# evenrose/CMDIAD

Measured on AMD Instinct MI355X. Metric: images/sec end-to-end (extract+distill+kNN score), higher is better.
Workload: dtype bf16; 1 GPU; configs[1]: DINO ViT-B/8 + Point-MAE predict (DoubleRGBPointFeatures: both modalities are extracted, this method has no distillation step at test time; the `mtfi_step` leg times the method that has one), 224x224 RGB + 24576-point clouds (1024 groups x 128), batch 32/GPU, bagel-sized banks (xyz 76518x768, rgb 19129x768); batch_per_gpu=32, rotating_input_batches=4, bank=single, hip_graphs=True, search_operands=bf16 (fp32 accumulate, exact fp32 re-score of the winner), weights=seeded random init (no checkpoints offline)

## Files before the change

### cmdiad_amd/csrc/mlp_fused.hip

```cpp
#include "gemm_core.h"
#include "launch.h"

namespace {

using namespace gemm;

constexpr int kC = 384, kHid = 1536, kBM = 128, kWaves = 8;
constexpr int kChunks = kHid / 64;
constexpr int kKT1 = kC / BK;
constexpr int kPer = kKT1 + kC / 64;
constexpr int kSlots = 6, kAhead = kSlots - 1;
static_assert(kPer % kSlots == 0, "the slot of a piece depends on its place in the chunk only");
constexpr int kPieceBytes = 64 * BK * 2;
constexpr int kXbWave = kKT1 * 16 * BK * 2;
constexpr int kHOff = kWaves * kXbWave;
constexpr int kRingOff = kHOff + kWaves * 2048;
constexpr int kLdsBytes = kRingOff + kSlots * kPieceBytes;
static_assert(kLdsBytes == 160 * 1024, "LDS budget");

struct MlpParams {
    int M;
    const bf16_t* xb;
    const float* row_scale;
    const bf16_t* w1;
    const float* b1;
    const bf16_t* w2;
    const float* b2;
    float* x;
    bf16_t* ln_xb;
    float* ln_part;
    const float* add2;
};

__device__ __forceinline__ void mlp_barrier() { asm volatile("s_barrier" ::: "memory"); }

__device__ __forceinline__ float half_row_sum8(float v)
{
    v += __builtin_bit_cast(float, __builtin_amdgcn_update_dpp(0, __builtin_bit_cast(int, v), 0xB1, 0xF, 0xF, false));
    v += __builtin_bit_cast(float, __builtin_amdgcn_update_dpp(0, __builtin_bit_cast(int, v), 0x4E, 0xF, 0xF, false));
    v += __builtin_bit_cast(float, __builtin_amdgcn_update_dpp(0, __builtin_bit_cast(int, v), 0x141, 0xF, 0xF, false));
    return v;
}

template <bool LN_OUT>
__global__ __launch_bounds__(512, 1) void pmae_mlp_fused_kernel(MlpParams p)
{
    extern __shared__ __attribute__((aligned(16))) char lds[];
    const int lane = threadIdx.x & 63, wave = __builtin_amdgcn_readfirstlane(threadIdx.x >> 6);
    const int g = lane >> 4, r16 = lane & 15;
    const int mw = (int)blockIdx.x * kBM + wave * 16;
    char* xs = lds + wave * kXbWave;
    char* hs = lds + kHOff + wave * 2048;
    char* ring = lds + kRingOff;

    float rsc;
    f32x4 b1v[4];
    auto load_b1 = [&](int c) {
        const float* bp = p.b1 + c * 64 + g * 4;
#pragma unroll
        for (int j = 0; j < 4; ++j) asm volatile("global_load_dwordx4 %0, %1, off" : "=v"(b1v[j]) : "v"(bp + j * 16) : "memory");
    };
    {
        const float* rp = p.row_scale + min(mw + r16, p.M - 1);
        asm volatile("global_load_dword %0, %1, off" : "=v"(rsc) : "v"(rp) : "memory");
    }
    load_b1(0);
    const int sw_chunk = (lane & 7) ^ (lane >> 3);
#pragma unroll
    for (int e = 0; e < 2; ++e) {
        const bf16_t* src = p.xb + (size_t)min(mw + e * 8 + (lane >> 3), p.M - 1) * kC + sw_chunk * 8;
#pragma unroll
        for (int s = 0; s < kKT1; ++s)
            __builtin_amdgcn_global_load_lds((const __attribute__((address_space(1))) void*)(src + s * BK),
                                             (__attribute__((address_space(3))) void*)(xs + s * 2048 + e * 1024), 16, 0, 0);
    }
    const char* w1l = reinterpret_cast<const char*>(p.w1 + (size_t)(wave * 8 + (lane >> 3)) * kC + sw_chunk * 8);
    const char* w2l = reinterpret_cast<const char*>(p.w2 + (size_t)(wave * 8 + (lane >> 3)) * kHid + sw_chunk * 8);
    auto issue = [&](int c, int q) {
        const char* src = q < kKT1 ? w1l + ((size_t)c * 64 * kC + q * BK) * 2 : w2l + ((size_t)(q - kKT1) * 64 * kHid + c * BK) * 2;
        __builtin_amdgcn_global_load_lds((const __attribute__((address_space(1))) void*)src,
                                         (__attribute__((address_space(3))) void*)(ring + (q % kSlots) * kPieceBytes + wave * 1024), 16, 0, 0);
    };
#pragma unroll
    for (int q = 0; q < kAhead; ++q) issue(0, q);
    asm volatile("s_waitcnt vmcnt(4)" ::: "memory");
    mlp_barrier();

    auto ldf = [&](const char* tile, int row, int kk) { return *reinterpret_cast<const bf16x8*>(tile + lds_off(row, kk * 4 + g)); };
    auto step = [&](const char* wt, const bf16x8& a0, const bf16x8& a1, f32x4 (&acc)[4]) {
        bf16x8 wf[2][4];
#pragma unroll
        for (int kk = 0; kk < 2; ++kk)
#pragma unroll
            for (int j = 0; j < 4; ++j) wf[kk][j] = ldf(wt, j * 16 + r16, kk);
        __builtin_amdgcn_s_setprio(1);
#pragma unroll
        for (int kk = 0; kk < 2; ++kk)
#pragma unroll
            for (int j = 0; j < 4; ++j) acc[j] = mfma16(wf[kk][j], kk ? a1 : a0, acc[j]);
        __builtin_amdgcn_s_setprio(0);
    };

    f32x4 acc2[kC / 64][4];
#pragma unroll
    for (int nb = 0; nb < kC / 64; ++nb)
#pragma unroll
        for (int j = 0; j < 4; ++j) acc2[nb][j] = f32x4{0.f, 0.f, 0.f, 0.f};

    for (int c = 0; c < kChunks; ++c) {
        f32x4 acc1[4];
#pragma unroll
        for (int j = 0; j < 4; ++j) acc1[j] = f32x4{0.f, 0.f, 0.f, 0.f};
        bf16x8 h0, h1;
#pragma unroll
        for (int q = 0; q < kPer; ++q) {
            const int qn = q + kAhead < kPer ? q + kAhead : q + kAhead - kPer;
            const int cn = q + kAhead < kPer ? c : c + 1;
            const bool more = cn < kChunks;
            if (q == 7 && more) load_b1(c + 1);
            if (more) issue(cn, qn);
            const char* wt = ring + (q % kSlots) * kPieceBytes;
            if (q < kKT1) step(wt, ldf(xs + q * 2048, r16, 0), ldf(xs + q * 2048, r16, 1), acc1);
            else step(wt, h0, h1, acc2[q - kKT1]);
            if (!more) asm volatile("s_waitcnt vmcnt(0)" ::: "memory");
            else if (q >= 7 && q <= 10) asm volatile("s_waitcnt vmcnt(8)" ::: "memory");
            else asm volatile("s_waitcnt vmcnt(4)" ::: "memory");
            mlp_barrier();
            if (q == kKT1 - 1) {
                __builtin_amdgcn_sched_barrier(0);
#pragma unroll
                for (int j = 0; j < 4; ++j) {
                    f32x4 v = __builtin_elementwise_fma(acc1[j], f32x4{rsc, rsc, rsc, rsc}, b1v[j]);
                    v = gelu_erf4(v);
                    const bf16x4 hv = {f2bf(v[0]), f2bf(v[1]), f2bf(v[2]), f2bf(v[3])};
                    *reinterpret_cast<bf16x4*>(hs + lds_off(r16, 2 * j + (g >> 1)) + (g & 1) * 8) = hv;
                }
                h0 = ldf(hs, r16, 0);
                h1 = ldf(hs, r16, 1);
            }
        }
    }

    RowStore32 rs;
    rs.init(hs, lane);
    const bool full = mw + 16 <= p.M;
    const int m0r = mw + rs.R;
    const int ma = min(m0r, p.M - 1), mb = min(m0r + 8, p.M - 1);
#pragma unroll
    for (int nb = 0; nb < kC / 64; ++nb) {
        const int n0 = nb * 64;
        f32x4 bj[4];
#pragma unroll
        for (int j = 0; j < 4; ++j) bj[j] = *reinterpret_cast<const f32x4*>(p.b2 + n0 + j * 16 + g * 4);
        f32x4 o0[2], o1[2];
#pragma unroll
        for (int ch = 0; ch < 2; ++ch) {
            const int col = n0 + ch * 32 + rs.u * 4;
            const f32x4 r0 = *reinterpret_cast<const f32x4*>(p.x + (size_t)ma * kC + col);
            const f32x4 r1 = *reinterpret_cast<const f32x4*>(p.x + (size_t)mb * kC + col);
            f32x4 a0 = {0.f, 0.f, 0.f, 0.f}, a1 = a0;
            if (LN_OUT && p.add2) {
                a0 = *reinterpret_cast<const f32x4*>(p.add2 + (size_t)ma * kC + col);
                a1 = *reinterpret_cast<const f32x4*>(p.add2 + (size_t)mb * kC + col);
            }
            rs.park(acc2[nb][2 * ch] + bj[2 * ch], acc2[nb][2 * ch + 1] + bj[2 * ch + 1]);
            f32x4 t0, t1;
            rs.fetch(t0, t1);
            o0[ch] = t0 + r0;
            o1[ch] = t1 + r1;
            if (LN_OUT && p.add2) { o0[ch] += a0; o1[ch] += a1; }
            if (full || m0r < p.M) *reinterpret_cast<f32x4*>(p.x + (size_t)m0r * kC + col) = o0[ch];
            if (full || m0r + 8 < p.M) *reinterpret_cast<f32x4*>(p.x + (size_t)(m0r + 8) * kC + col) = o1[ch];
            if constexpr (LN_OUT) {
                const bf16x4 v0 = {f2bf(o0[ch][0]), f2bf(o0[ch][1]), f2bf(o0[ch][2]), f2bf(o0[ch][3])};
                const bf16x4 v1 = {f2bf(o1[ch][0]), f2bf(o1[ch][1]), f2bf(o1[ch][2]), f2bf(o1[ch][3])};
                if (full || m0r < p.M) *reinterpret_cast<bf16x4*>(p.ln_xb + (size_t)m0r * kC + col) = v0;
                if (full || m0r + 8 < p.M) *reinterpret_cast<bf16x4*>(p.ln_xb + (size_t)(m0r + 8) * kC + col) = v1;
            }
        }
        if constexpr (LN_OUT) {
            float s0 = 0.f, s1 = 0.f;
#pragma unroll
            for (int ch = 0; ch < 2; ++ch)
#pragma unroll
                for (int q = 0; q < 4; ++q) { s0 += o0[ch][q]; s1 += o1[ch][q]; }
            s0 = half_row_sum8(s0);
            s1 = half_row_sum8(s1);
            const float c0 = s0 * (1.0f / 64), c1 = s1 * (1.0f / 64);
            float q0 = 0.f, q1 = 0.f;
#pragma unroll
            for (int ch = 0; ch < 2; ++ch)
#pragma unroll
                for (int q = 0; q < 4; ++q) {
                    const float d0 = o0[ch][q] - c0, d1 = o1[ch][q] - c1;
                    q0 = fmaf(d0, d0, q0);
                    q1 = fmaf(d1, d1, q1);
                }
            q0 = half_row_sum8(q0);
            q1 = half_row_sum8(q1);
            if (rs.u == 0) {
                float2* part = reinterpret_cast<float2*>(p.ln_part) + (size_t)nb * p.M;
                if (full || m0r < p.M) part[m0r] = make_float2(s0, q0);
                if (full || m0r + 8 < p.M) part[m0r + 8] = make_float2(s1, q1);
            }
        }
    }
}

}

int cmdiad_pmae_mlp_fused(float* x, const uint16_t* xb, const float* rstd, const uint16_t* w1, const float* b1, const uint16_t* w2,
                          const float* b2, int M, uint16_t* ln_xb, float* ln_part, const float* add2, cmdiad_stream_t stream)
{
    CMDIAD_REQUIRE(x && xb && rstd && w1 && b1 && w2 && b2 && M > 0, CMDIAD_ERR_ARG, "cmdiad_pmae_mlp_fused: null operand");
    CMDIAD_REQUIRE(aligned16(x) && aligned16(xb) && aligned16(w1) && aligned16(w2) && aligned16(b1) && aligned16(b2) && (!add2 || aligned16(add2)), CMDIAD_ERR_ARG,
                   "cmdiad_pmae_mlp_fused: operands must be 16-byte aligned");
    CMDIAD_REQUIRE(!ln_xb == !ln_part && (ln_xb || !add2) && (!ln_xb || (((uintptr_t)ln_xb & 7) == 0 && ((uintptr_t)ln_part & 7) == 0)),
                   CMDIAD_ERR_ARG, "cmdiad_pmae_mlp_fused: ln_xb and ln_part come together (8-byte aligned); add2 only with them");
    MlpParams p{M, (const bf16_t*)xb, rstd, (const bf16_t*)w1, b1, (const bf16_t*)w2, b2, x, (bf16_t*)ln_xb, ln_part, add2};
    const dim3 grid((unsigned)((M + kBM - 1) / kBM)), block(kWaves * 64);
    const int rc = ln_xb ? launch_lds<pmae_mlp_fused_kernel<true>>("cmdiad_pmae_mlp_fused", grid, block, kLdsBytes, (hipStream_t)stream, p)
                         : launch_lds<pmae_mlp_fused_kernel<false>>("cmdiad_pmae_mlp_fused", grid, block, kLdsBytes, (hipStream_t)stream, p);
    if (rc) return rc;
    CMDIAD_CHECK_LAUNCH();
    return CMDIAD_OK;
}
```

Measured before the change: 1581 images/s.

## Retile fused Point-MAE MLP into 32x32 wave tiles with double-buffered fragments

Changes the fused FC1-GELU-FC2 kernel so that each wave owns a 32-row by half-width tile instead of 16 full-width rows. The input and hidden tiles become shared across the block, and FC2 output columns are split between wave pairs. The change also double-buffers LDS fragment reads against MFMAs, issues two weight pieces per phase through explicit SGPR-based DMA, and adds lgkmcnt waits before each barrier. The aim is to cut per-MFMA LDS weight traffic and hide LDS latency. In exchange it needs an extra barrier for the shared hidden tile and takes on more register pressure and a trickier ring-slot schedule.

```diff
diff --git a/cmdiad_amd/csrc/mlp_fused.hip b/cmdiad_amd/csrc/mlp_fused.hip
--- a/cmdiad_amd/csrc/mlp_fused.hip
+++ b/cmdiad_amd/csrc/mlp_fused.hip
@@ -9,14 +9,16 @@
 constexpr int kChunks = kHid / 64;
 constexpr int kKT1 = kC / BK;
 constexpr int kPer = kKT1 + kC / 64;
-constexpr int kSlots = 6, kAhead = kSlots - 1;
+constexpr int kSlots = 6;
 static_assert(kPer % kSlots == 0, "the slot of a piece depends on its place in the chunk only");
 constexpr int kPieceBytes = 64 * BK * 2;
-constexpr int kXbWave = kKT1 * 16 * BK * 2;
-constexpr int kHOff = kWaves * kXbWave;
-constexpr int kRingOff = kHOff + kWaves * 2048;
+constexpr int kXbBlock = kBM * BK * 2;
+constexpr int kHOff = kKT1 * kXbBlock;
+constexpr int kHBytes = kBM * 64 * 2;
+constexpr int kRingOff = kHOff + kHBytes;
 constexpr int kLdsBytes = kRingOff + kSlots * kPieceBytes;
 static_assert(kLdsBytes == 160 * 1024, "LDS budget");
+static_assert(kHBytes >= kWaves * 2048, "the hidden tile doubles as the waves' RowStore32 scratch");
 
 struct MlpParams {
     int M;
@@ -32,7 +34,7 @@
     const float* add2;
 };
 
-__device__ __forceinline__ void mlp_barrier() { asm volatile("s_barrier" ::: "memory"); }
+__device__ __forceinline__ void mlp_barrier() { asm volatile("s_waitcnt lgkmcnt(0)\n\ts_barrier" ::: "memory"); }
 
 __device__ __forceinline__ float half_row_sum8(float v)
 {
@@ -48,160 +50,214 @@
     extern __shared__ __attribute__((aligned(16))) char lds[];
     const int lane = threadIdx.x & 63, wave = __builtin_amdgcn_readfirstlane(threadIdx.x >> 6);
     const int g = lane >> 4, r16 = lane & 15;
-    const int mw = (int)blockIdx.x * kBM + wave * 16;
-    char* xs = lds + wave * kXbWave;
-    char* hs = lds + kHOff + wave * 2048;
+    const int tr = wave >> 1, nc = wave & 1;
+    const int m0 = (int)blockIdx.x * kBM;
+    const int mt = m0 + tr * 32;
+    char* xs = lds;
+    char* hs = lds + kHOff;
     char* ring = lds + kRingOff;
 
-    float rsc;
-    f32x4 b1v[4];
+    float rsc[2];
+    f32x4 b1v[2];
     auto load_b1 = [&](int c) {
-        const float* bp = p.b1 + c * 64 + g * 4;
-#pragma unroll
-        for (int j = 0; j < 4; ++j) asm volatile("global_load_dwordx4 %0, %1, off" : "=v"(b1v[j]) : "v"(bp + j * 16) : "memory");
-    };
+        const float* bp = p.b1 + c * 64 + nc * 32 + g * 4;
+#pragma unroll
+        for (int j = 0; j < 2; ++j) asm volatile("global_load_dwordx4 %0, %1, off" : "=v"(b1v[j]) : "v"(bp + j * 16) : "memory");
+    };
+#pragma unroll
+    for (int i = 0; i < 2; ++i) {
+        const float* rp = p.row_scale + min(mt + i * 16 + r16, p.M - 1);
+        asm volatile("global_load_dword %0, %1, off" : "=v"(rsc[i]) : "v"(rp) : "memory");
+    }
+    load_b1(0);
+    auto dma = [&](const char* ubase, unsigned voff, unsigned lds_addr) {
+        unsigned long long sb;
+        asm volatile("s_mov_b64 %0, %2\n\ts_mov_b32 m0, %3\n\ts_nop 0\n\tglobal_load_lds_dwordx4 %1, %0"
+                     : "=&s"(sb) : "v"(voff), "s"(ubase), "s"(lds_addr) : "memory");
+    };
+    const unsigned lds0 = (unsigned)(size_t)(__attribute__((address_space(3))) char*)lds;
+    const unsigned pch = (unsigned)(((lane & 7) ^ (lane >> 3)) * 16);
     {
-        const float* rp = p.row_scale + min(mw + r16, p.M - 1);
-        asm volatile("global_load_dword %0, %1, off" : "=v"(rsc) : "v"(rp) : "memory");
-    }
-    load_b1(0);
-    const int sw_chunk = (lane & 7) ^ (lane >> 3);
-#pragma unroll
-    for (int e = 0; e < 2; ++e) {
-        const bf16_t* src = p.xb + (size_t)min(mw + e * 8 + (lane >> 3), p.M - 1) * kC + sw_chunk * 8;
-#pragma unroll
-        for (int s = 0; s < kKT1; ++s)
-            __builtin_amdgcn_global_load_lds((const __attribute__((address_space(1))) void*)(src + s * BK),
-                                             (__attribute__((address_space(3))) void*)(xs + s * 2048 + e * 1024), 16, 0, 0);
-    }
-    const char* w1l = reinterpret_cast<const char*>(p.w1 + (size_t)(wave * 8 + (lane >> 3)) * kC + sw_chunk * 8);
-    const char* w2l = reinterpret_cast<const char*>(p.w2 + (size_t)(wave * 8 + (lane >> 3)) * kHid + sw_chunk * 8);
+        const char* xb0 = reinterpret_cast<const char*>(p.xb) + (size_t)m0 * kC * 2;
+        const int last = p.M - 1 - m0;
+#pragma unroll
+        for (int e = 0; e < 2; ++e) {
+            const unsigned voff = (unsigned)min(wave * 16 + e * 8 + (lane >> 3), last) * (unsigned)(kC * 2) + pch;
+#pragma unroll
+            for (int s = 0; s < kKT1; ++s) dma(xb0 + s * BK * 2, voff, lds0 + s * kXbBlock + (wave * 16 + e * 8) * 128);
+        }
+    }
+    const unsigned off1 = (unsigned)(wave * 8 + (lane >> 3)) * (unsigned)(kC * 2) + pch;
+    const unsigned off2 = (unsigned)(wave * 8 + (lane >> 3)) * (unsigned)(kHid * 2) + pch;
     auto issue = [&](int c, int q) {
-        const char* src = q < kKT1 ? w1l + ((size_t)c * 64 * kC + q * BK) * 2 : w2l + ((size_t)(q - kKT1) * 64 * kHid + c * BK) * 2;
-        __builtin_amdgcn_global_load_lds((const __attribute__((address_space(1))) void*)src,
-                                         (__attribute__((address_space(3))) void*)(ring + (q % kSlots) * kPieceBytes + wave * 1024), 16, 0, 0);
-    };
-#pragma unroll
-    for (int q = 0; q < kAhead; ++q) issue(0, q);
+        const unsigned dst = lds0 + kRingOff + (q % kSlots) * kPieceBytes + wave * 1024;
+        if (q < kKT1) dma(reinterpret_cast<const char*>(p.w1) + ((size_t)c * 64 * kC + q * BK) * 2, off1, dst);
+        else dma(reinterpret_cast<const char*>(p.w2) + ((size_t)(q - kKT1) * 64 * kHid + c * BK) * 2, off2, dst);
+    };
+#pragma unroll
+    for (int q = 0; q < kSlots; ++q) issue(0, q);
     asm volatile("s_waitcnt vmcnt(4)" ::: "memory");
     mlp_barrier();
 
     auto ldf = [&](const char* tile, int row, int kk) { return *reinterpret_cast<const bf16x8*>(tile + lds_off(row, kk * 4 + g)); };
-    auto step = [&](const char* wt, const bf16x8& a0, const bf16x8& a1, f32x4 (&acc)[4]) {
-        bf16x8 wf[2][4];
+    bf16x8 fx[2][2][2];
+    bf16x8 fw[2][4];
+    bf16x8 hf[2][2];
+    f32x4 acc1[2][2];
+    f32x4 acc2[3][2][4];
+    auto read_fc1 = [&](int h, int s) {
+        const char* xt = xs + s * kXbBlock;
+        const char* wt = ring + s * kPieceBytes;
+#pragma unroll
+        for (int kk = 0; kk < 2; ++kk) {
+#pragma unroll
+            for (int i = 0; i < 2; ++i) fx[h][kk][i] = ldf(xt, tr * 32 + i * 16 + r16, kk);
+#pragma unroll
+            for (int jj = 0; jj < 2; ++jj) fw[h][2 * kk + jj] = ldf(wt, nc * 32 + jj * 16 + r16, kk);
+        }
+    };
+    auto mfma_fc1 = [&](int h) {
+        __builtin_amdgcn_s_setprio(1);
 #pragma unroll
         for (int kk = 0; kk < 2; ++kk)
 #pragma unroll
-            for (int j = 0; j < 4; ++j) wf[kk][j] = ldf(wt, j * 16 + r16, kk);
+            for (int i = 0; i < 2; ++i)
+#pragma unroll
+                for (int jj = 0; jj < 2; ++jj) acc1[i][jj] = mfma16(fw[h][2 * kk + jj], fx[h][kk][i], acc1[i][jj]);
+        __builtin_amdgcn_s_setprio(0);
+    };
+    auto read_fc2 = [&](int kk, int pp) {
+        const char* wt = ring + (2 * pp + nc) * kPieceBytes;
+#pragma unroll
+        for (int j = 0; j < 4; ++j) fw[kk][j] = ldf(wt, j * 16 + r16, kk);
+    };
+    auto mfma_fc2 = [&](int kk, int pp) {
         __builtin_amdgcn_s_setprio(1);
 #pragma unroll
-        for (int kk = 0; kk < 2; ++kk)
-#pragma unroll
-            for (int j = 0; j < 4; ++j) acc[j] = mfma16(wf[kk][j], kk ? a1 : a0, acc[j]);
+        for (int i = 0; i < 2; ++i)
+#pragma unroll
+            for (int j = 0; j < 4; ++j) acc2[pp][i][j] = mfma16(fw[kk][j], hf[kk][i], acc2[pp][i][j]);
         __builtin_amdgcn_s_setprio(0);
     };
 
-    f32x4 acc2[kC / 64][4];
-#pragma unroll
-    for (int nb = 0; nb < kC / 64; ++nb)
-#pragma unroll
-        for (int j = 0; j < 4; ++j) acc2[nb][j] = f32x4{0.f, 0.f, 0.f, 0.f};
-
+#pragma unroll
+    for (int pp = 0; pp < 3; ++pp)
+#pragma unroll
+        for (int i = 0; i < 2; ++i)
+#pragma unroll
+            for (int j = 0; j < 4; ++j) acc2[pp][i][j] = f32x4{0.f, 0.f, 0.f, 0.f};
+
+    read_fc1(0, 0);
     for (int c = 0; c < kChunks; ++c) {
-        f32x4 acc1[4];
-#pragma unroll
-        for (int j = 0; j < 4; ++j) acc1[j] = f32x4{0.f, 0.f, 0.f, 0.f};
-        bf16x8 h0, h1;
-#pragma unroll
-        for (int q = 0; q < kPer; ++q) {
-            const int qn = q + kAhead < kPer ? q + kAhead : q + kAhead - kPer;
-            const int cn = q + kAhead < kPer ? c : c + 1;
-            const bool more = cn < kChunks;
-            if (q == 7 && more) load_b1(c + 1);
-            if (more) issue(cn, qn);
-            const char* wt = ring + (q % kSlots) * kPieceBytes;
-            if (q < kKT1) step(wt, ldf(xs + q * 2048, r16, 0), ldf(xs + q * 2048, r16, 1), acc1);
-            else step(wt, h0, h1, acc2[q - kKT1]);
-            if (!more) asm volatile("s_waitcnt vmcnt(0)" ::: "memory");
-            else if (q >= 7 && q <= 10) asm volatile("s_waitcnt vmcnt(8)" ::: "memory");
-            else asm volatile("s_waitcnt vmcnt(4)" ::: "memory");
+        const bool more = c + 1 < kChunks;
+#pragma unroll
+        for (int i = 0; i < 2; ++i)
+#pragma unroll
+            for (int jj = 0; jj < 2; ++jj) acc1[i][jj] = f32x4{0.f, 0.f, 0.f, 0.f};
+#pragma unroll
+        for (int P = 0; P < 6; ++P) {
+            if (P < 3) { read_fc1(1, 2 * P + 1); __builtin_amdgcn_sched_barrier(0); mfma_fc1(0); }
+            else { read_fc2(1, P - 3); __builtin_amdgcn_sched_barrier(0); mfma_fc2(0, P - 3); }
+            if (P >= 4 && !more) asm volatile("s_waitcnt vmcnt(0)" ::: "memory");
+            else if (P == 4) asm volatile("s_waitcnt vmcnt(4)" ::: "memory");
+            else asm volatile("s_waitcnt vmcnt(2)" ::: "memory");
             mlp_barrier();
-            if (q == kKT1 - 1) {
+            if (P < 3) { issue(c, 2 * P + 6); issue(c, 2 * P + 7); }
+            else if (more) {
+                if (P == 3) load_b1(c + 1);
+                issue(c + 1, 2 * P - 6);
+                issue(c + 1, 2 * P - 5);
+            }
+            if (P < 2) { read_fc1(0, 2 * P + 2); __builtin_amdgcn_sched_barrier(0); mfma_fc1(1); }
+            else if (P == 2) {
+                mfma_fc1(1);
                 __builtin_amdgcn_sched_barrier(0);
 #pragma unroll
-                for (int j = 0; j < 4; ++j) {
-                    f32x4 v = __builtin_elementwise_fma(acc1[j], f32x4{rsc, rsc, rsc, rsc}, b1v[j]);
-                    v = gelu_erf4(v);
-                    const bf16x4 hv = {f2bf(v[0]), f2bf(v[1]), f2bf(v[2]), f2bf(v[3])};
-                    *reinterpret_cast<bf16x4*>(hs + lds_off(r16, 2 * j + (g >> 1)) + (g & 1) * 8) = hv;
+                for (int i = 0; i < 2; ++i)
+#pragma unroll
+                    for (int jj = 0; jj < 2; ++jj) {
+                        f32x4 v = __builtin_elementwise_fma(acc1[i][jj], f32x4{rsc[i], rsc[i], rsc[i], rsc[i]}, b1v[jj]);
+                        v = gelu_erf4(v);
+                        const bf16x4 hv = {f2bf(v[0]), f2bf(v[1]), f2bf(v[2]), f2bf(v[3])};
+                        *reinterpret_cast<bf16x4*>(hs + lds_off(tr * 32 + i * 16 + r16, 4 * nc + 2 * jj + (g >> 1)) + (g & 1) * 8) = hv;
+                    }
+                mlp_barrier();
+#pragma unroll
+                for (int kk = 0; kk < 2; ++kk)
+#pragma unroll
+                    for (int i = 0; i < 2; ++i) hf[kk][i] = ldf(hs, tr * 32 + i * 16 + r16, kk);
+                read_fc2(0, 0);
+            } else if (P < 5) { read_fc2(0, P - 2); __builtin_amdgcn_sched_barrier(0); mfma_fc2(1, P - 3); }
+            else { read_fc1(0, 0); __builtin_amdgcn_sched_barrier(0); mfma_fc2(1, 2); }
+        }
+    }
+
+    RowStore32 rs;
+    rs.init(hs + wave * 2048, lane);
+#pragma unroll
+    for (int i = 0; i < 2; ++i) {
+        const int mw = mt + i * 16;
+        const bool full = mw + 16 <= p.M;
+        const int m0r = mw + rs.R;
+        const int ma = min(m0r, p.M - 1), mb = min(m0r + 8, p.M - 1);
+#pragma unroll
+        for (int pp = 0; pp < 3; ++pp) {
+            const int nb = 2 * pp + nc;
+            const int n0 = nb * 64;
+            f32x4 bj[4];
+#pragma unroll
+            for (int j = 0; j < 4; ++j) bj[j] = *reinterpret_cast<const f32x4*>(p.b2 + n0 + j * 16 + g * 4);
+            f32x4 o0[2], o1[2];
+#pragma unroll
+            for (int ch = 0; ch < 2; ++ch) {
+                const int col = n0 + ch * 32 + rs.u * 4;
+                const f32x4 r0 = *reinterpret_cast<const f32x4*>(p.x + (size_t)ma * kC + col);
+                const f32x4 r1 = *reinterpret_cast<const f32x4*>(p.x + (size_t)mb * kC + col);
+                f32x4 a0 = {0.f, 0.f, 0.f, 0.f}, a1 = a0;
+                if (LN_OUT && p.add2) {
+                    a0 = *reinterpret_cast<const f32x4*>(p.add2 + (size_t)ma * kC + col);
+                    a1 = *reinterpret_cast<const f32x4*>(p.add2 + (size_t)mb * kC + col);
                 }
-                h0 = ldf(hs, r16, 0);
-                h1 = ldf(hs, r16, 1);
+                rs.park(acc2[pp][i][2 * ch] + bj[2 * ch], acc2[pp][i][2 * ch + 1] + bj[2 * ch + 1]);
+                f32x4 t0, t1;
+                rs.fetch(t0, t1);
+                o0[ch] = t0 + r0;
+                o1[ch] = t1 + r1;
+                if (LN_OUT && p.add2) { o0[ch] += a0; o1[ch] += a1; }
+                if (full || m0r < p.M) *reinterpret_cast<f32x4*>(p.x + (size_t)m0r * kC + col) = o0[ch];
+                if (full || m0r + 8 < p.M) *reinterpret_cast<f32x4*>(p.x + (size_t)(m0r + 8) * kC + col) = o1[ch];
+                if constexpr (LN_OUT) {
+                    const bf16x4 v0 = {f2bf(o0[ch][0]), f2bf(o0[ch][1]), f2bf(o0[ch][2]), f2bf(o0[ch][3])};
+                    const bf16x4 v1 = {f2bf(o1[ch][0]), f2bf(o1[ch][1]), f2bf(o1[ch][2]), f2bf(o1[ch][3])};
+                    if (full || m0r < p.M) *reinterpret_cast<bf16x4*>(p.ln_xb + (size_t)m0r * kC + col) = v0;
+                    if (full || m0r + 8 < p.M) *reinterpret_cast<bf16x4*>(p.ln_xb + (size_t)(m0r + 8) * kC + col) = v1;
+                }
             }
-        }
-    }
-
-    RowStore32 rs;
-    rs.init(hs, lane);
-    const bool full = mw + 16 <= p.M;
-    const int m0r = mw + rs.R;
-    const int ma = min(m0r, p.M - 1), mb = min(m0r + 8, p.M - 1);
-#pragma unroll
-    for (int nb = 0; nb < kC / 64; ++nb) {
-        const int n0 = nb * 64;
-        f32x4 bj[4];
-#pragma unroll
-        for (int j = 0; j < 4; ++j) bj[j] = *reinterpret_cast<const f32x4*>(p.b2 + n0 + j * 16 + g * 4);
-        f32x4 o0[2], o1[2];
-#pragma unroll
-        for (int ch = 0; ch < 2; ++ch) {
-            const int col = n0 + ch * 32 + rs.u * 4;
-            const f32x4 r0 = *reinterpret_cast<const f32x4*>(p.x + (size_t)ma * kC + col);
-            const f32x4 r1 = *reinterpret_cast<const f32x4*>(p.x + (size_t)mb * kC + col);
-            f32x4 a0 = {0.f, 0.f, 0.f, 0.f}, a1 = a0;
-            if (LN_OUT && p.add2) {
-                a0 = *reinterpret_cast<const f32x4*>(p.add2 + (size_t)ma * kC + col);
-                a1 = *reinterpret_cast<const f32x4*>(p.add2 + (size_t)mb * kC + col);
-            }
-            rs.park(acc2[nb][2 * ch] + bj[2 * ch], acc2[nb][2 * ch + 1] + bj[2 * ch + 1]);
-            f32x4 t0, t1;
-            rs.fetch(t0, t1);
-            o0[ch] = t0 + r0;
-            o1[ch] = t1 + r1;
-            if (LN_OUT && p.add2) { o0[ch] += a0; o1[ch] += a1; }
-            if (full || m0r < p.M) *reinterpret_cast<f32x4*>(p.x + (size_t)m0r * kC + col) = o0[ch];
-            if (full || m0r + 8 < p.M) *reinterpret_cast<f32x4*>(p.x + (size_t)(m0r + 8) * kC + col) = o1[ch];
             if constexpr (LN_OUT) {
-                const bf16x4 v0 = {f2bf(o0[ch][0]), f2bf(o0[ch][1]), f2bf(o0[ch][2]), f2bf(o0[ch][3])};
-                const bf16x4 v1 = {f2bf(o1[ch][0]), f2bf(o1[ch][1]), f2bf(o1[ch][2]), f2bf(o1[ch][3])};
-                if (full || m0r < p.M) *reinterpret_cast<bf16x4*>(p.ln_xb + (size_t)m0r * kC + col) = v0;
-                if (full || m0r + 8 < p.M) *reinterpret_cast<bf16x4*>(p.ln_xb + (size_t)(m0r + 8) * kC + col) = v1;
-            }
-        }
-        if constexpr (LN_OUT) {
-            float s0 = 0.f, s1 = 0.f;
-#pragma unroll
-            for (int ch = 0; ch < 2; ++ch)
-#pragma unroll
-                for (int q = 0; q < 4; ++q) { s0 += o0[ch][q]; s1 += o1[ch][q]; }
-            s0 = half_row_sum8(s0);
-            s1 = half_row_sum8(s1);
-            const float c0 = s0 * (1.0f / 64), c1 = s1 * (1.0f / 64);
-            float q0 = 0.f, q1 = 0.f;
-#pragma unroll
-            for (int ch = 0; ch < 2; ++ch)
-#pragma unroll
-                for (int q = 0; q < 4; ++q) {
-                    const float d0 = o0[ch][q] - c0, d1 = o1[ch][q] - c1;
-                    q0 = fmaf(d0, d0, q0);
-                    q1 = fmaf(d1, d1, q1);
+                float s0 = 0.f, s1 = 0.f;
+#pragma unroll
+                for (int ch = 0; ch < 2; ++ch)
+#pragma unroll
+                    for (int q = 0; q < 4; ++q) { s0 += o0[ch][q]; s1 += o1[ch][q]; }
+                s0 = half_row_sum8(s0);
+                s1 = half_row_sum8(s1);
+                const float c0 = s0 * (1.0f / 64), c1 = s1 * (1.0f / 64);
+                float q0 = 0.f, q1 = 0.f;
+#pragma unroll
+                for (int ch = 0; ch < 2; ++ch)
+#pragma unroll
+                    for (int q = 0; q < 4; ++q) {
+                        const float d0 = o0[ch][q] - c0, d1 = o1[ch][q] - c1;
+                        q0 = fmaf(d0, d0, q0);
+                        q1 = fmaf(d1, d1, q1);
+                    }
+                q0 = half_row_sum8(q0);
+                q1 = half_row_sum8(q1);
+                if (rs.u == 0) {
+                    float2* part = reinterpret_cast<float2*>(p.ln_part) + (size_t)nb * p.M;
+                    if (full || m0r < p.M) part[m0r] = make_float2(s0, q0);
+                    if (full || m0r + 8 < p.M) part[m0r + 8] = make_float2(s1, q1);
                 }
-            q0 = half_row_sum8(q0);
-            q1 = half_row_sum8(q1);
-            if (rs.u == 0) {
-                float2* part = reinterpret_cast<float2*>(p.ln_part) + (size_t)nb * p.M;
-                if (full || m0r < p.M) part[m0r] = make_float2(s0, q0);
-                if (full || m0r + 8 < p.M) part[m0r + 8] = make_float2(s1, q1);
             }
         }
     }
```

Result: no change. 1584 images/s (median of 4 runs) (+0.2%).
